# deryrahman/image-caption-emotion-indonesia

Measured on AMD Instinct MI355X. Metric: images/sec (train step) + NLL loss match, batch=64 ResNet152+FactoredLSTM-512, higher is better.
Workload: dtype f32 (trunk: operands as 2 f16 pieces each, 3 MFMA products per multiply, f32 accumulate; decoder: large products as 3 bf16 pieces per operand, 6 MFMA products per multiply, the rest f32 MFMA; the persistent LSTM kernel the trunk's split-f16 scheme)

## Files before the change

image-caption-emotion-indonesia_amd/_lib.py:

```python
import ctypes as C
import os

_HERE = os.path.dirname(os.path.abspath(__file__))
LIB_PATH = os.path.join(_HERE, "libcapnet_hip.so")

_f = C.POINTER(C.c_float)
_vp = C.c_void_p
_i = C.c_int
_l = C.c_long
_sz = C.c_size_t
_ip = C.POINTER(C.c_int)

SIGNATURES = {
    "capnet_last_error": (C.c_char_p, []),
    "capnet_abi_version": (_i, []),
    "capnet_sgemm": (_i, [_i, _i, _i, _i, _i, _vp, _l, _vp, _l, _vp, _l, _vp, _i, _i, _l, _l, _l,
                          _l, _i, _vp]),
    "capnet_sgemm_b3": (_i, [_i, _i, _i, _i, _i, _vp, _l, _vp, _l, _vp, _l, _vp, _i, _i, _l, _l, _l, _l, _vp, _sz, _vp]),
    "capnet_sgemm_b3_eligible": (_i, [_i, _i, _i, _i, _i, _vp, _l, _vp, _l, _vp, _l, _vp, _i, _l, _l, _l, _l]),
    "capnet_sgemm_splitk": (_i, [_i, _i, _i, _i, _i, _vp, _l, _vp, _l, _vp, _l, _vp, _i, _vp, _sz, _vp]),
    "capnet_sgemm_splitk_fused": (_i, [_i, _i, _i, _i, _i, _vp, _l, _vp, _l, _vp, _l, _vp, _i, _vp, _sz, _vp, _sz, _vp]),
    "capnet_colsum": (_i, [_vp, _l, _i, _i, _vp, _i, _vp]),
    "capnet_argmax_rows": (_i, [_vp, _i, _i, _i, _vp, _vp]),
    "capnet_resize_u8": (_i, [_vp, _i, _i, _vp, _vp, _i, _i, _vp, _vp, _i, _vp, _vp, _i, _vp]),
# ... 38 lines not shown
    "capnet_conv1x1_f16x3_weight_words": (_sz, [_i, _i]),
    "capnet_conv1x1_f16x3_bn": (_i, [_l, _i]),
    "capnet_conv1x1_f16x3_pack": (_i, [_vp, _vp, _i, _i, _i, _vp]),
    "capnet_conv1x1_fwd_f16x3": (_i, [_vp, _l, _l, _l, _vp, _i, _vp, _vp, _vp, _i, _vp, _vp, _i, _i, _i, _i, _i,
                                      _i, _vp, _vp, _vp, _i, _vp]),
    "capnet_conv3x3_fwd_patch": (_i, [_vp, _vp, _i, _vp, _vp, _vp, _i, _vp, _vp, _i, _i, _i, _i, _i, _i, _vp]),
    "capnet_conv1x1_fwd_tail": (_i, [_vp, _vp, _vp, _vp, _vp, _vp, _vp, _vp, _i, _vp, _vp, _vp, _l, _i, _i, _vp]),
    "capnet_conv2d_fwd_f16x3_scaled": (_i, [_vp, _l, _l, _l, _vp, _i, _vp, _vp, _vp, _i, _vp, _vp, _i, _i, _i, _i, _i,
                                            _i, _i, _i, _i, _vp]),
    "capnet_conv3x3_fwd_patch_scaled": (_i, [_vp, _vp, _i, _vp, _vp, _vp, _i, _vp, _vp, _i, _i, _i, _i, _i, _i, _i, _vp]),
    "capnet_conv1x1_fwd_tail_scaled": (_i, [_vp, _vp, _vp, _vp, _vp, _vp, _vp, _vp, _i, _vp, _vp, _vp, _l, _i, _i, _i, _vp]),
    "capnet_conv_stem_f16x3_weight_words": (_sz, []),
    "capnet_conv_stem_f16x3_part_rows": (_i, [_i, _i, _i]),
    "capnet_conv_stem_f16x3_pack": (_i, [_vp, _vp, _vp]),
    "capnet_conv_stem_fwd_f16x3": (_i, [_vp, _l, _l, _l, _vp, _vp, _vp, _vp, _i, _i, _i, _vp]),
    "capnet_conv_f16x3_weight_words": (_sz, [_i, _i, _i]),
    "capnet_conv_f16x3_pack": (_i, [_vp, _vp, _i, _i, _i, _i, _vp]),
    "capnet_conv2d_fwd_f16x3": (_i, [_vp, _l, _l, _l, _vp, _i, _vp, _vp, _vp, _i, _vp, _vp, _i, _i, _i, _i, _i,
                                     _i, _i, _i, _vp, _vp, _vp, _i, _vp]),
    "capnet_conv_kmajor_slab_floats": (_sz, [_i, _i, _i, _i]),
    "capnet_conv_kmajor_plan": (None, [_i, _i, _i, _i, _ip]),
    "capnet_conv_kmajor_tiles_m": (_i, [_i, _i, _i, _i]),
    "capnet_conv_tiles_m": (_i, [_i, _i, _i]),
    "capnet_bn_finalize": (_i, [_vp, _vp, _i, _i, _l, _vp, _vp, _vp, _vp, C.c_float, C.c_float,
                                _vp, _vp, _vp]),
    "capnet_bn_add_relu": (_i, [_vp, _vp, _vp, _vp, _vp, _vp, _vp, _l, _i, _vp]),
    "capnet_bn_relu_maxpool": (_i, [_vp, _vp, _vp, _vp, _i, _i, _i, _i, _vp]),
    "capnet_global_avgpool": (_i, [_vp, _vp, _i, _i, _i, _vp]),
    "capnet_bn1d_fwd": (_i, [_vp, _i, _i, _vp, _vp, _vp, _vp, _i, C.c_float, C.c_float, _vp, _vp,
                             _vp, _vp]),
# ... 210 lines not shown
```

image-caption-emotion-indonesia_amd/csrc/capi.cpp:

```cpp
#include "../../include/capnet.h"

#include "common.h"
#include "kernels.h"

using namespace capnet;

static inline hipStream_t S(capnet_stream_t s) { return reinterpret_cast<hipStream_t>(s); }

static SeqDims to_dims(const int* d) {
  SeqDims r;
  r.B = d[0]; r.T = d[1]; r.steps = d[2]; r.N = d[3]; r.E = d[4]; r.F = d[5]; r.H = d[6];
  r.V = d[7]; r.has_features = d[8]; r.cell = d[9];
  return r;
}

static bool weight_used(int cell, int i) { return cell == kCellFactored || i == 0 || i == 4 || i == 24 || i == 28; }
template <class Weights>
static void to_weights(const float* const* weights, Weights& w) {
  for (int g = 0; g < 4; ++g) {
    w.Vw[g] = weights[0 + g];  w.Vb[g] = weights[4 + g];
    w.Sw[g] = weights[8 + g];  w.Sb[g] = weights[12 + g];
    w.Uw[g] = weights[16 + g]; w.Ub[g] = weights[20 + g];
    w.Ww[g] = weights[24 + g]; w.Wb[g] = weights[28 + g];
  }
// ... 137 lines not shown
}
int capnet_conv1x1_fwd_tail_scaled(const float* y3, const float* s1, const float* t1, const float* res, const float* s2,
                                   const float* t2, float* tail_out, const unsigned* image, int bn, float* y,
                                   float* part_sum, float* part_sq, long M, int Cin, int Cout, int in_exp,
                                   capnet_stream_t stream) {
  return conv1x1_fwd_tail(y3, s1, t1, res, s2, t2, tail_out, image, bn, y, part_sum, part_sq, M, Cin, Cout, S(stream), in_exp);
}
size_t capnet_conv_stem_f16x3_weight_words(void) { return conv_stem_f16x3_weight_words(); }
int capnet_conv_stem_f16x3_part_rows(int B, int H, int W) { return conv_stem_f16x3_part_rows(B, H, W); }
int capnet_conv_stem_f16x3_pack(const float* w_oihw, unsigned* image, capnet_stream_t stream) {
  return conv_stem_f16x3_pack(w_oihw, image, S(stream));
}
int capnet_conv_stem_fwd_f16x3(const float* x, long sxb, long sxc, long sxh, const unsigned* image, float* y,
                               float* part_sum, float* part_sq, int B, int H, int W, capnet_stream_t stream) {
  return conv_stem_fwd_f16x3(x, sxb, sxc, sxh, image, y, part_sum, part_sq, B, H, W, S(stream));
}

int capnet_sgemm_splitk(int transA, int transB, int M, int N, int K, const float* A, long lda,
                        const float* B, long ldb, float* C, long ldc, const float* bias,
                        int accumulate, float* workspace, size_t workspace_floats,
                        capnet_stream_t stream) {
  CAPNET_REQUIRE(M >= 0 && N >= 0 && K >= 0, "sgemm_splitk: negative dimension");
  return sgemm_splitk(transA != 0, transB != 0, M, N, K, A, lda, B, ldb, C, ldc, bias, accumulate,
                      workspace, workspace_floats, S(stream));
}
int capnet_sgemm_splitk_fused(int transA, int transB, int M, int N, int K, const float* A, long lda,
                              const float* B, long ldb, float* C, long ldc, const float* bias,
                              int accumulate, float* workspace, size_t workspace_floats, int* counters,
                              size_t n_counters, capnet_stream_t stream) {
  CAPNET_REQUIRE(M >= 0 && N >= 0 && K >= 0, "sgemm_splitk_fused: negative dimension");
// ... 1083 lines not shown
```

image-caption-emotion-indonesia_amd/csrc/conv_stem.hip:

```cpp
#include <cstdlib>

#include "common.h"
#include "mfma_core.h"
#include "split_f16.h"
#include "kernels.h"

namespace capnet {
namespace {

constexpr int kRows = 22;
constexpr int kSteps = kRows / 2;
constexpr int kSeg = 128;
constexpr int kCols = 2 * kSeg + 8;
constexpr int kGroups = kCols / 4;
constexpr int kRowDw = 160;
constexpr int kPlane = kRows * kRowDw * 4;
constexpr int kImgBytes = 2 * kSteps * 2 * 64 * 16;
constexpr int kLoads = (21 * kGroups + 255) / 256;
constexpr int kWgs = 512;
static_assert(kRowDw * 2 >= kCols && kRowDw % 64 == 32, "staged row stride");

struct StemArgs {
  const float* x;
  const unsigned* wimg;
  float* y;
  float* part_sum;
  float* part_sq;
  int B, H, W, OH, OW, chunks, tiles, in_exp;
  int* err;
  int sxb, sxc, sxh;
  unsigned tile_mul, tile_sh;
  unsigned oh_mul, oh_sh;
};

__global__ __launch_bounds__(256, 2) void conv_stem_f16x3_kernel(const StemArgs g) {
  __shared__ __attribute__((aligned(16))) unsigned char lds[kImgBytes + 2 * kPlane];
  __shared__ float s_red[2][4][64];
  unsigned char* const wl = lds;
  unsigned char* const xl = lds + kImgBytes;
  const int tid = threadIdx.x, lane = tid & 63, wave = tid >> 6;
  const int li = lane & 31, lh = lane >> 5;
  const float oscale = f16x3_out_scale(g.wimg[0], g.in_exp);
  const float iscale = ldexpf(1.f, g.in_exp);

  {
    const u4* src = reinterpret_cast<const u4*>(g.wimg + kF16x3HdrWords);
    for (int i = tid; i < kImgBytes / 16; i += 256) *reinterpret_cast<u4*>(wl + i * 16) = src[i];
    for (int i = tid; i < kRowDw; i += 256) {
      *reinterpret_cast<unsigned*>(xl + (21 * kRowDw + i) * 4) = 0u;
      *reinterpret_cast<unsigned*>(xl + kPlane + (21 * kRowDw + i) * 4) = 0u;
    }
  }

  f32x4 pre[kLoads];
  auto fetch = [&](int tile) {
    const int boh = (int)fast_div((unsigned)tile, g.tile_mul, g.tile_sh), chunk = tile - boh * g.chunks;
    const int b = (int)fast_div((unsigned)boh, g.oh_mul, g.oh_sh), oh = boh - b * g.OH;
    const int iw0 = 2 * chunk * kSeg - 4;
#pragma unroll
    for (int u = 0; u < kLoads; ++u) {
      const int i = tid + 256 * u;
      const int r = i / kGroups, q = i - r * kGroups;
      const int c = r / 7, kh = r - 7 * c;
      const int ih = 2 * oh - 3 + kh, iw = iw0 + 4 * q;
      const bool ok = r < 21 && (unsigned)ih < (unsigned)g.H && iw >= 0 && iw < g.W;
      f32x4 v = {0.f, 0.f, 0.f, 0.f};
      if (ok) v = *reinterpret_cast<const f32x4*>(g.x + (long)b * g.sxb + (long)c * g.sxc + (long)ih * g.sxh + iw);
      pre[u] = v;
    }
  };
  auto stage = [&]() {
#pragma unroll
    for (int u = 0; u < kLoads; ++u) {
      const int i = tid + 256 * u;
      const int r = i / kGroups, q = i - r * kGroups;
      if (r < 21) {
        h4 h, l;
        split4(pre[u] * iscale, h, l);
        *reinterpret_cast<h4*>(xl + r * kRowDw * 4 + q * 8) = h;
        *reinterpret_cast<h4*>(xl + kPlane + r * kRowDw * 4 + q * 8) = l;
      }
    }
  };

  float csum[2] = {0.f, 0.f}, csq[2] = {0.f, 0.f};
  const int G = (int)gridDim.x;
  int tile = xcd_remap((int)blockIdx.x, G);
  if (tile < g.tiles) fetch(tile);
  __syncthreads();
  for (; tile < g.tiles; tile += G) {
    stage();
    __syncthreads();
    const int boh = (int)fast_div((unsigned)tile, g.tile_mul, g.tile_sh), chunk = tile - boh * g.chunks;
    if (tile + G < g.tiles) fetch(tile + G);
    f32x16 acc[2];
#pragma unroll
    for (int nb = 0; nb < 2; ++nb)
#pragma unroll
      for (int r = 0; r < 16; ++r) acc[nb][r] = 0.f;
    const unsigned char* arow = xl + (lh * kRowDw + 32 * wave + li) * 4;
    const unsigned char* brow = wl + (lh * 64 + li) * 16;
#pragma unroll
    for (int s = 0; s < kSteps; ++s) {
      h8 a[2], bf[2][2];
#pragma unroll
      for (int p = 0; p < 2; ++p) {
        const unsigned* ap = reinterpret_cast<const unsigned*>(arow + p * kPlane + s * 2 * kRowDw * 4);
        const u4 av = {ap[0], ap[1], ap[2], ap[3]};
        a[p] = __builtin_bit_cast(h8, av);
#pragma unroll
        for (int nb = 0; nb < 2; ++nb)
          bf[p][nb] = *reinterpret_cast<const h8*>(brow + ((p * kSteps + s) * 2 * 64 + nb * 32) * 16);
      }
#pragma unroll
      for (int nb = 0; nb < 2; ++nb) {
        acc[nb] = __builtin_amdgcn_mfma_f32_32x32x16_f16(a[1], bf[0][nb], acc[nb], 0, 0, 0);
        acc[nb] = __builtin_amdgcn_mfma_f32_32x32x16_f16(a[0], bf[1][nb], acc[nb], 0, 0, 0);
        acc[nb] = __builtin_amdgcn_mfma_f32_32x32x16_f16(a[0], bf[0][nb], acc[nb], 0, 0, 0);
      }
    }
    const int ow_base = chunk * kSeg + 32 * wave + 4 * lh;
    float* yrow = g.y + ((long)boh * g.OW) * 64;
#pragma unroll
    for (int nb = 0; nb < 2; ++nb) {
#pragma unroll
      for (int r = 0; r < 16; ++r) {
        const int ow = ow_base + (r & 3) + 8 * (r >> 2);
        const float v = acc[nb][r] * oscale;
        if (ow < g.OW) {
          yrow[(long)ow * 64 + nb * 32 + li] = v;
          csum[nb] += v;
          csq[nb] = fmaf(v, v, csq[nb]);
        }
      }
    }
    __syncthreads();
  }
  if (!g.part_sum && g.err) flag_nonfinite(csq[0] + csq[1], g.err);
  if (g.part_sum) {
#pragma unroll
    for (int nb = 0; nb < 2; ++nb) {
      csum[nb] += __shfl_xor(csum[nb], 32);
      csq[nb] += __shfl_xor(csq[nb], 32);
      if (lh == 0) {
        s_red[0][wave][nb * 32 + li] = csum[nb];
        s_red[1][wave][nb * 32 + li] = csq[nb];
      }
    }
    __syncthreads();
    if (tid < 64) {
      g.part_sum[(long)blockIdx.x * 64 + tid] = (s_red[0][0][tid] + s_red[0][1][tid]) + (s_red[0][2][tid] + s_red[0][3][tid]);
// ... 58 lines not shown
                        float* part_sq, int Bn, int H, int W, hipStream_t stream, int in_exp, int* err) {
  CAPNET_REQUIRE(x && wimg && y && aligned16(wimg) && in_exp > -64 && in_exp < 64, "conv_stem_fwd_f16x3: bad argument");
  CAPNET_REQUIRE(conv_stem_f16x3_eligible(x, sxb, sxc, sxh, 1, Bn, H, W, 3, 64, 7, 2, 3),
                 "conv_stem_fwd_f16x3: operands not eligible (B=%d %dx%d)", Bn, H, W);
  CAPNET_REQUIRE((part_sum == nullptr) == (part_sq == nullptr), "conv_stem_fwd_f16x3: stats pair");
  StemArgs a{};
  a.x = x; a.wimg = wimg; a.y = y; a.part_sum = part_sum; a.part_sq = part_sq;
  a.B = Bn; a.H = H; a.W = W; a.OH = (H - 1) / 2 + 1; a.OW = (W - 1) / 2 + 1;
  a.in_exp = in_exp; a.err = err;
  a.chunks = cdiv(a.OW, kSeg);
  a.tiles = Bn * a.OH * a.chunks;
  a.sxb = (int)sxb; a.sxc = (int)sxc; a.sxh = (int)sxh;
  magic_div((unsigned)a.chunks, &a.tile_mul, &a.tile_sh);
  magic_div((unsigned)a.OH, &a.oh_mul, &a.oh_sh);
  const int grid = a.tiles < kWgs ? a.tiles : kWgs;
  CAPNET_LAUNCH_TIMED(conv_stem_f16x3_kernel, dim3(grid), dim3(256), stream, a);
  CAPNET_LAUNCH_CHECK();
  return kOk;
}

}
```

image-caption-emotion-indonesia_amd/csrc/kernels.h:

```cpp
#pragma once
#include <hip/hip_runtime.h>

namespace capnet {

int sgemm(bool ta, bool tb, int M, int N, int K, const float* A, long lda, const float* B,
          long ldb, float* C, long ldc, const float* bias, int accumulate, int batch, long sA,
          long sB, long sC, long sBias, int force_tile, hipStream_t stream);

bool sgemm_b3_eligible(bool ta, bool tb, int M, int N, int K, const float* A, long lda, const float* B, long ldb,
                       const float* C, long ldc, const float* bias, int batch, long sA, long sB, long sC, long sBias);
int sgemm_b3(bool ta, bool tb, int M, int N, int K, const float* A, long lda, const float* B, long ldb, float* C, long ldc,
             const float* bias, int accumulate, int batch, long sA, long sB, long sC, long sBias, hipStream_t stream,
             float* ws = nullptr, size_t ws_floats = 0);

constexpr size_t kSplitKCounters = 1024;
int sgemm_splitk(bool ta, bool tb, int M, int N, int K, const float* A, long lda, const float* B,
                 long ldb, float* C, long ldc, const float* bias, int accumulate, float* ws,
                 size_t ws_floats, hipStream_t stream, int* counters = nullptr, size_t n_counters = 0);
int sgemm_splitk_slabs(bool tb, int M, int N, int K, const float* A, long lda, const float* B, long ldb,
                       float* ws, size_t ws_floats, int* n_slabs, hipStream_t stream);
int sgemm_rows16_slabs(bool tb, int M, int N, int K, const float* A, long lda, const float* B, long ldb, float* ws,
                       size_t ws_floats, int* n_slabs, hipStream_t stream);
int sgemm_splitk_batched(bool ta, bool tb, int M, int N, int K, const float* A, long lda,
                         const float* B, long ldb, float* C, long ldc, const float* bias,
// ... 37 lines not shown
size_t conv_f16x3_weight_words(int Cin, int Cout, int k);
int f16x3_pack_header(const float* w, unsigned* img, long n, hipStream_t stream);
int conv_f16x3_pack(const float* w_oihw, unsigned* img, int Cout, int Cin, int k, int bn, hipStream_t stream);
int conv_fwd_f16x3(const float* x, long sxb, long sxh, long sxw, const unsigned* wimg, int bn, float* y,
                   const float* in_scale, const float* in_shift, int relu_in, float* part_sum, float* part_sq, int Bn,
                   int H, int W, int Cin, int Cout, int k, int stride, int pad, hipStream_t stream,
                   const float* out_scale = nullptr, const float* out_shift = nullptr, const float* res = nullptr,
                   int relu_out = 0, int in_exp = 0, int* err = nullptr);
bool conv_stem_f16x3_eligible(const float* x, long sxb, long sxc, long sxh, long sxw, int Bn, int H, int W, int Cin,
                              int Cout, int k, int stride, int pad);
size_t conv_stem_f16x3_weight_words();
int conv_stem_f16x3_part_rows(int Bn, int H, int W);
int conv_stem_f16x3_pack(const float* w_oihw, unsigned* img, hipStream_t stream);
int conv_stem_fwd_f16x3(const float* x, long sxb, long sxc, long sxh, const unsigned* wimg, float* y, float* part_sum,
                        float* part_sq, int Bn, int H, int W, hipStream_t stream, int in_exp = 0, int* err = nullptr);
bool conv3x3_patch_eligible(const float* x, long sxb, long sxh, long sxw, long sxc, int Bn, int H, int W, int Cin,
                            int Cout, int k, int stride, int pad, const float* in_scale, const float* in_shift);
int conv3x3_fwd_patch(const float* x, const unsigned* wimg, int bn, float* y, const float* in_scale, const float* in_shift,
                      int relu_in, float* part_sum, float* part_sq, int Bn, int H, int W, int Cin, int Cout,
                      hipStream_t stream, bool shared_chip = false, int in_exp = 0, int* err = nullptr);
bool conv1x1_areg_eligible(const float* x, long M, int Cin, int Cout, int bn, const float* in_scale, const float* in_shift);
int conv1x1_fwd_areg(const float* x, const unsigned* wimg, int bn, float* y, const float* in_scale, const float* in_shift,
                     int relu_in, float* part_sum, float* part_sq, long M, int Cin, int Cout, int in_exp, hipStream_t stream,
                     int* err = nullptr);
bool conv1x1_tail_eligible(const float* y3, const float* res, long M, int Cin, int Cout);
int conv1x1_fwd_tail(const float* y3, const float* s1, const float* t1, const float* res, const float* s2, const float* t2,
                     float* tail_out, const unsigned* wimg, int bn, float* y, float* part_sum, float* part_sq, long M,
                     int Cin, int Cout, hipStream_t stream, int in_exp = 0, int* err = nullptr);
size_t conv1x1_f16x3_weight_words(int Cin, int Cout);
int conv1x1_f16x3_pack(const float* w, unsigned* img, int Cout, int Cin, int bn, hipStream_t stream);
// ... 382 lines not shown
```

image-caption-emotion-indonesia_amd/csrc/trunk.cpp:

```cpp
#include <algorithm>
#include <cstdint>
#include <cstdlib>
#include <cstring>
#include <cstdio>
#include <utility>
#include <vector>

#include "common.h"
#include "kernels.h"

namespace capnet {

struct TrunkConv {
  int Cin, Cout, k, stride, pad;
  int H, W;
  int OH, OW;
  int Kw;
  bool kmajor;
  bool h3;
  int tile_n;
  bool stem_h3 = false;
  bool fused3 = false, fused1 = false;
};

// ... 1 lines not shown
  int stage, index;
  int i1, i2, i3, id;
};

struct Trunk {
  int B, H, W;
  std::vector<TrunkConv> convs;
  std::vector<TrunkBlock> blocks;
  size_t off_x[2], off_y1, off_y2, off_y3, off_d, off_part, off_slab, off_gram, off_ss, total_floats;
  std::vector<size_t> ss_off;
  std::vector<size_t> bs_off;
  int final_side;
  bool tail_balance = true;
  bool use_patch = true, fuse_tails = true, use_areg = false;
  int fused_stages = 0;
  bool timing = false;
  int timing_every = 1;
  long pass_no = 0;
  bool timing_now = false;
  bool timing_once = false;
  std::vector<hipEvent_t> ev_pool;
  size_t ev_next = 0;
  std::vector<hipEvent_t> ev;
  double timed_flops = 0;
};

static int round_up(int v, int m) { return (v + m - 1) / m * m; }
static const float* const kAlignedDummy = reinterpret_cast<const float*>(uintptr_t(256));

int trunk_create(int B, int H, int W, Trunk** out) {
// ... 68 lines not shown
      max_y1 = std::max(max_y1, (size_t)c1.OH * c1.OW * c1.Cout);
      max_y2 = std::max(max_y2, (size_t)c2.OH * c2.OW * c2.Cout);
      max_y3 = std::max(max_y3, (size_t)c3.OH * c3.OW * c3.Cout);
      t->blocks.push_back(TrunkBlock{L, b, i1, i1 + 1, i1 + 2, b == 0 ? i1 + 3 : -1});
      if (b == 0) {
        TrunkConv d = add(inplanes, p * 4, 1, stride, 0, h, w, true);
        max_d = std::max(max_d, (size_t)d.OH * d.OW * d.Cout);
      }
      h = c2.OH; w = c2.OW;
      inplanes = p * 4;
      max_x = std::max(max_x, (size_t)h * w * inplanes);
    }
  }
  t->final_side = h;
  CAPNET_REQUIRE(h == w, "trunk_create: only square feature maps are supported");
  max_y3 = std::max(max_y3, (size_t)stem.OH * stem.OW * 64);
  size_t off = 0;
  auto take = [&](size_t n) { size_t o = off; off += (n + 63) / 64 * 64; return o; };
  t->off_x[0] = take(max_x * B);
  t->off_x[1] = take(max_x * B);
  t->off_y1 = take(max_y1 * B);
  t->off_y2 = take(max_y2 * B);
  t->off_y3 = take(max_y3 * B);
  t->off_d = take(max_d * B);
  size_t max_part = 0;
  for (auto& c : t->convs) {
    const long M = (long)B * c.OH * c.OW;
    const int tile = c.kmajor ? conv_v2_auto_tile((int)M, c.Cout, c.Kw) : conv_auto_tile((int)M, c.Cout);
    max_part = std::max(max_part, (size_t)conv_tiles_m((int)M, tile) * c.Cout);
    if (c.h3) max_part = std::max(max_part, (size_t)conv1x1_tiles_m(M) * c.Cout);
    if (c.stem_h3) max_part = std::max(max_part, (size_t)conv_stem_f16x3_part_rows(B, c.H, c.W) * c.Cout);
  }
  max_part = std::max(max_part, max_fpart);
  t->off_part = take(2 * max_part);
  size_t max_slab = 0;
  for (auto& c : t->convs)
    if (c.kmajor) max_slab = std::max(max_slab, conv_v2_slab_floats(B * c.OH * c.OW, c.Cout, c.Kw, 0));
  t->off_slab = take(max_slab + 64);
  t->off_gram = take(max_gram + 64);
  t->off_ss = off;
  for (auto& c : t->convs) t->ss_off.push_back(take(2 * (size_t)c.Cout));
  for (auto& c : t->convs) t->bs_off.push_back(take(2 * (size_t)c.Cout));
  t->total_floats = off;
  *out = t;
  return kOk;
}
// ... 187 lines not shown
int conv_bn(const Ctx& c, int i, const float* x, long sxb, long sxh, long sxw, long sxc,
            const float* in_scale, const float* in_shift, int relu_in, float* y, const BlockTail* tail = nullptr) {
  const TrunkConv& d = c.t->convs[i];
  const long M = (long)c.t->B * d.OH * d.OW;
  CAPNET_REQUIRE(d.tile_n != 256 || d.k == 3 || (tail && (c.train || c.eval_ready)), "trunk: conv %d was planned for the wide tail kernel", i);
  const bool fuse_tail = tail && (c.train || c.eval_ready) && c.t->fuse_tails && d.h3 && d.k == 1 && d.stride == 1 && !in_scale &&
                         x == tail->out && tail->C == d.Cin && tail->rows == M && sxc == 1 && sxw == d.Cin &&
                         sxh == (long)d.W * d.Cin && sxb == (long)d.H * d.W * d.Cin &&
                         conv1x1_tail_eligible(tail->y3, tail->res, M, d.Cin, d.Cout);
  if (tail && !fuse_tail) {
    const int rt = run_tail(c, *tail);
    if (rt) return rt;
  }
  int tile = d.kmajor ? conv_v2_auto_tile((int)M, d.Cout, d.Kw) : conv_auto_tile((int)M, d.Cout);
  if (d.kmajor && !c.t->tail_balance && M >= 5000) tile = 12864;
  const int prows = d.stem_h3 ? conv_stem_f16x3_part_rows(c.t->B, d.H, d.W) : d.h3 ? conv1x1_tiles_m(M) : conv_tiles_m((int)M, tile);
  float* psum = c.ws + c.t->off_part;
  float* psq = psum + (size_t)prows * d.Cout;
  const bool attach = fuse_tail || d.stem_h3 || d.h3;
  const int rc = timed_launch(c.t, attach, c.s, trunk_conv_flops(c.t, i), [&]() -> int {
    const unsigned* wimg = reinterpret_cast<const unsigned*>(c.w[i]);
    float* ps = c.train ? psum : nullptr;
    float* pq = c.train ? psq : nullptr;
    if (fuse_tail)
      return conv1x1_fwd_tail(tail->y3, tail->s1, tail->t1, tail->res, tail->s2, tail->t2, tail->out, wimg, d.tile_n, y, ps, pq, M,
                              d.Cin, d.Cout, c.s, c.in_exp(i), c.err);
    if (d.stem_h3) {
      CAPNET_REQUIRE(!in_scale && conv_stem_f16x3_eligible(x, sxb, sxc, sxh, sxw, c.t->B, d.H, d.W, d.Cin, d.Cout, d.k, d.stride, d.pad),
                     "trunk: the stem is planned for the split-f16 kernel but its operands are not eligible");
      return conv_stem_fwd_f16x3(x, sxb, sxc, sxh, wimg, y, ps, pq, c.t->B, d.H, d.W, c.s, c.in_exp(i), c.err);
    }
    if (d.h3 && d.k == 3 && c.t->use_patch &&
        conv3x3_patch_eligible(x, sxb, sxh, sxw, sxc, c.t->B, d.H, d.W, d.Cin, d.Cout, d.k, d.stride, d.pad, in_scale, in_shift))
      return conv3x3_fwd_patch(x, wimg, d.tile_n, y, in_scale, in_shift, relu_in, ps, pq, c.t->B, d.H, d.W, d.Cin, d.Cout, c.s,
                               !c.t->tail_balance, c.in_exp(i), c.err);
    if (d.h3 && d.k == 1 && d.stride == 1 && c.t->use_areg && sxc == 1 && sxw == d.Cin && sxh == (long)d.W * d.Cin &&
        sxb == (long)d.H * d.W * d.Cin && conv1x1_areg_eligible(x, M, d.Cin, d.Cout, d.tile_n, in_scale, in_shift))
      return conv1x1_fwd_areg(x, wimg, d.tile_n, y, in_scale, in_shift, relu_in, ps, pq, M, d.Cin, d.Cout, c.in_exp(i), c.s, c.err);
    if (d.h3) {
      CAPNET_REQUIRE(conv_f16x3_eligible(x, sxb, sxh, sxw, sxc, c.t->B, d.H, d.W, d.Cin, d.Cout, d.k, d.stride, d.pad, in_scale, in_shift),
                     "trunk: conv %d planned for the split-f16 kernel but its operands are not eligible", i);
      return conv_fwd_f16x3(x, sxb, sxh, sxw, wimg, d.tile_n, y, in_scale, in_shift, relu_in, ps, pq, c.t->B, d.H, d.W, d.Cin, d.Cout,
                            d.k, d.stride, d.pad, c.s, nullptr, nullptr, nullptr, 0, c.in_exp(i), c.err);
    }
// ... 153 lines not shown
  float* Y1 = workspace + t->off_y1;
  float* Y2 = workspace + t->off_y2;
  float* Y3 = workspace + t->off_y3;
  float* D = workspace + t->off_d;
  int rc;
  if (!train) {
    const char* fe = getenv("CAPNET_EVAL_FOLDED");
    if (fe && fe[0] == '1') return trunk_forward_eval(c, images_nchw, out_pooled, out_map);
    rc = eval_scale_shift_all(c);
    if (rc) return rc;
    c.eval_ready = true;
  }
  {
    const TrunkConv& d = t->convs[0];
    rc = conv_bn(c, 0, images_nchw, (long)3 * d.H * d.W, d.W, 1, (long)d.H * d.W, nullptr,
                 nullptr, 0, Y3);
    if (rc) return rc;
    rc = bn_relu_maxpool(Y3, c.scale(0), c.shift(0), X[0], B, d.OH, d.OW, 64, stream);
    if (rc) return rc;
  }
  int cur = 0;
  BlockTail tail{};
  FusedTail ftail{};
  bool have_tail = false, have_ftail = false;
  for (const TrunkBlock& blk : t->blocks) {
    const int i1 = blk.i1, i2 = blk.i2, i3 = blk.i3, id = blk.id;
    const TrunkConv& c1 = t->convs[i1];
    const TrunkConv& c2 = t->convs[i2];
    const TrunkConv& c3 = t->convs[i3];
    const float* x = X[cur];
    float* out = X[cur ^ 1];
    auto nhwc = [](const TrunkConv& d, long* sb, long* sh, long* sw) {
      *sw = d.Cin; *sh = (long)d.W * d.Cin; *sb = (long)d.H * d.W * d.Cin;
    };
    long sb, sh, sw;
    nhwc(c1, &sb, &sh, &sw);
    if (have_ftail) {
      CAPNET_REQUIRE(c1.fused1 && (c.train || c.eval_ready), "trunk: conv %d is not the fused boundary the plan made", i1);
      rc = fused_conv1_bn(c, i1, ftail, Y1);
      have_ftail = false;
    } else {
      CAPNET_REQUIRE(!c1.fused1, "trunk: conv %d was planned for fused_block.hip", i1);
      rc = conv_bn(c, i1, x, sb, sh, sw, 1, nullptr, nullptr, 0, Y1, have_tail ? &tail : nullptr);
    }
    have_tail = false;
    if (rc) return rc;
    nhwc(c2, &sb, &sh, &sw);
    rc = conv_bn(c, i2, Y1, sb, sh, sw, 1, c.scale(i1), c.shift(i1), 1, Y2);
    if (rc) return rc;
    const long rows = (long)B * c3.OH * c3.OW;
    if (c3.fused3 && (c.train || c.eval_ready)) {
      rc = fused_stats_bn(c, i3, Y2, c.scale(i2), c.shift(i2));
      if (rc) return rc;
      if (id >= 0) {
        const TrunkConv& cd = t->convs[id];
        nhwc(cd, &sb, &sh, &sw);
        rc = conv_bn(c, id, x, sb, sh, sw, 1, nullptr, nullptr, 0, D);
        if (rc) return rc;
        ftail = FusedTail{i3, Y2, c.scale(i2), c.shift(i2), D, c.scale(id), c.shift(id), out};
      } else {
        ftail = FusedTail{i3, Y2, c.scale(i2), c.shift(i2), x, nullptr, nullptr, out};
      }
      have_ftail = true;
      cur ^= 1;
      continue;
    }
    CAPNET_REQUIRE(!c3.fused3, "trunk: conv %d was planned for fused_block.hip (the folded inference trunk must be chosen before the plan is made)", i3);
    nhwc(c3, &sb, &sh, &sw);
    rc = conv_bn(c, i3, Y2, sb, sh, sw, 1, c.scale(i2), c.shift(i2), 1, Y3);
    if (rc) return rc;
    if (id >= 0) {
      const TrunkConv& cd = t->convs[id];
      nhwc(cd, &sb, &sh, &sw);
      rc = conv_bn(c, id, x, sb, sh, sw, 1, nullptr, nullptr, 0, D);
      if (rc) return rc;
      tail = BlockTail{Y3, c.scale(i3), c.shift(i3), D, c.scale(id), c.shift(id), out, rows, c3.Cout};
    } else {
      tail = BlockTail{Y3, c.scale(i3), c.shift(i3), x, nullptr, nullptr, out, rows, c3.Cout};
    }
    have_tail = true;
    cur ^= 1;
  }
  if (have_tail) {
    rc = run_tail(c, tail);
    if (rc) return rc;
  }
  const int side = t->final_side;
  if (out_pooled) {
    rc = global_avgpool(X[cur], out_pooled, B, side * side, 2048, stream, c.err);
// ... 11 lines not shown
```

include/capnet.h:

```cpp
#ifndef CAPNET_H_
#define CAPNET_H_

#include <stddef.h>

#ifdef __cplusplus
extern "C" {
#endif

typedef void* capnet_stream_t;
typedef struct capnet_trunk capnet_trunk_t;

#define CAPNET_OK 0
#define CAPNET_ERR_INVALID_ARG (-1)
#define CAPNET_ERR_HIP (-2)

const char* capnet_last_error(void);
int capnet_abi_version(void);

int capnet_sgemm(int transA, int transB, int M, int N, int K, const float* A, long lda,
                 const float* B, long ldb, float* C, long ldc, const float* bias, int accumulate,
                 int batch, long strideA, long strideB, long strideC, long strideBias,
                 int force_tile, capnet_stream_t stream);
int capnet_sgemm_b3(int transA, int transB, int M, int N, int K, const float* A, long lda, const float* B, long ldb,
                    float* C, long ldc, const float* bias, int accumulate, int batch, long strideA, long strideB,
// ... 118 lines not shown
                                   float* part_sq, int B, int H, int W, int Cin, int Cout, int k, int stride, int pad,
                                   int in_exp, capnet_stream_t stream);
int capnet_conv3x3_fwd_patch_scaled(const float* x, const unsigned* image, int bn, float* y, const float* in_scale,
                                    const float* in_shift, int relu_in, float* part_sum, float* part_sq, int B, int H,
                                    int W, int Cin, int Cout, int shared_chip, int in_exp, capnet_stream_t stream);
int capnet_conv1x1_fwd_tail_scaled(const float* y3, const float* s1, const float* t1, const float* res, const float* s2,
                                   const float* t2, float* tail_out, const unsigned* image, int bn, float* y,
                                   float* part_sum, float* part_sq, long M, int Cin, int Cout, int in_exp,
                                   capnet_stream_t stream);

size_t capnet_conv_stem_f16x3_weight_words(void);
int capnet_conv_stem_f16x3_part_rows(int B, int H, int W);
int capnet_conv_stem_f16x3_pack(const float* w_oihw, unsigned* image, capnet_stream_t stream);
int capnet_conv_stem_fwd_f16x3(const float* x, long sxb, long sxc, long sxh, const unsigned* image, float* y,
                               float* part_sum, float* part_sq, int B, int H, int W, capnet_stream_t stream);

int capnet_conv2d_fwd_kmajor(const float* x, long sxb, long sxh, long sxw, const float* w_kmajor,
                             int k_rows, float* y, const float* in_scale, const float* in_shift,
                             int relu_in, float* part_sum, float* part_sq, int B, int H, int W,
                             int Cin, int Cout, int KH, int KW, int stride, int pad, int tile,
                             float* slabs, capnet_stream_t stream);
size_t capnet_conv_kmajor_slab_floats(int M, int Cout, int k_rows, int tile);
void capnet_conv_kmajor_plan(int M, int Cout, int k_rows, int tile, int* out5);
int capnet_conv_kmajor_tiles_m(int M, int Cout, int k_rows, int tile);
int capnet_conv_tiles_m(int M, int Cout, int tile);
int capnet_bn_finalize(const float* part_sum, const float* part_sq, int tiles, int C, long count,
                       const float* gamma, const float* beta, float* running_mean,
                       float* running_var, float momentum, float eps, float* scale, float* shift,
                       capnet_stream_t stream);
int capnet_bn_add_relu(const float* y, const float* s1, const float* t1, const float* res,
// ... 349 lines not shown
```

Measured before the change: 9208.

## Fuse stem conv with max-pool and defer BN-ReLU into first block convs

Adds a pooled variant of the split-f16 stem kernel that max-pools each output row pair in registers (sign-flipped by gamma so max commutes with the BN affine) and writes only the pooled map, while still gathering BN statistics. The separate BN+ReLU+maxpool pass and the full-resolution stem output round trip are dropped; the BN scale/shift and ReLU are instead applied on input by the first bottleneck's 1x1 and downsample convs. Work units are runs of pooled rows per image, which changes the stem's parallel decomposition and adds overlap rows and an extra LDS sync per row. It is on by default when eligible and can be disabled by env var. Forward trunk only.

```diff
diff --git a/image-caption-emotion-indonesia_amd/_lib.py b/image-caption-emotion-indonesia_amd/_lib.py
--- a/image-caption-emotion-indonesia_amd/_lib.py
+++ b/image-caption-emotion-indonesia_amd/_lib.py
@@ -76,6 +76,9 @@
     "capnet_conv_stem_f16x3_part_rows": (_i, [_i, _i, _i]),
     "capnet_conv_stem_f16x3_pack": (_i, [_vp, _vp, _vp]),
     "capnet_conv_stem_fwd_f16x3": (_i, [_vp, _l, _l, _l, _vp, _vp, _vp, _vp, _i, _i, _i, _vp]),
+    "capnet_conv_stem_pool_f16x3_eligible": (_i, [_vp, _l, _l, _l, _i, _i, _i]),
+    "capnet_conv_stem_pool_f16x3_part_rows": (_i, [_i, _i, _i]),
+    "capnet_conv_stem_pool_fwd_f16x3": (_i, [_vp, _l, _l, _l, _vp, _vp, _vp, _vp, _vp, _i, _i, _i, _i, _vp]),
     "capnet_conv_f16x3_weight_words": (_sz, [_i, _i, _i]),
     "capnet_conv_f16x3_pack": (_i, [_vp, _vp, _i, _i, _i, _i, _vp]),
     "capnet_conv2d_fwd_f16x3": (_i, [_vp, _l, _l, _l, _vp, _i, _vp, _vp, _vp, _i, _vp, _vp, _i, _i, _i, _i, _i,
diff --git a/image-caption-emotion-indonesia_amd/csrc/capi.cpp b/image-caption-emotion-indonesia_amd/csrc/capi.cpp
--- a/image-caption-emotion-indonesia_amd/csrc/capi.cpp
+++ b/image-caption-emotion-indonesia_amd/csrc/capi.cpp
@@ -175,6 +175,15 @@
 int capnet_conv_stem_fwd_f16x3(const float* x, long sxb, long sxc, long sxh, const unsigned* image, float* y,
                                float* part_sum, float* part_sq, int B, int H, int W, capnet_stream_t stream) {
   return conv_stem_fwd_f16x3(x, sxb, sxc, sxh, image, y, part_sum, part_sq, B, H, W, S(stream));
+}
+int capnet_conv_stem_pool_f16x3_eligible(const float* x, long sxb, long sxc, long sxh, int B, int H, int W) {
+  return conv_stem_pool_f16x3_eligible(x, sxb, sxc, sxh, 1, B, H, W, 3, 64, 7, 2, 3) ? 1 : 0;
+}
+int capnet_conv_stem_pool_f16x3_part_rows(int B, int H, int W) { return conv_stem_pool_f16x3_part_rows(B, H, W); }
+int capnet_conv_stem_pool_fwd_f16x3(const float* x, long sxb, long sxc, long sxh, const unsigned* image, const float* gamma,
+                                    float* pooled, float* part_sum, float* part_sq, int B, int H, int W, int in_exp,
+                                    capnet_stream_t stream) {
+  return conv_stem_pool_fwd_f16x3(x, sxb, sxc, sxh, image, gamma, pooled, part_sum, part_sq, B, H, W, S(stream), in_exp);
 }
 
 int capnet_sgemm_splitk(int transA, int transB, int M, int N, int K, const float* A, long lda,
diff --git a/image-caption-emotion-indonesia_amd/csrc/conv_stem.hip b/image-caption-emotion-indonesia_amd/csrc/conv_stem.hip
--- a/image-caption-emotion-indonesia_amd/csrc/conv_stem.hip
+++ b/image-caption-emotion-indonesia_amd/csrc/conv_stem.hip
@@ -18,6 +18,7 @@
 constexpr int kImgBytes = 2 * kSteps * 2 * 64 * 16;
 constexpr int kLoads = (21 * kGroups + 255) / 256;
 constexpr int kWgs = 512;
+constexpr int kPoolRun = 7;
 static_assert(kRowDw * 2 >= kCols && kRowDw % 64 == 32, "staged row stride");
 
 struct StemArgs {
@@ -31,11 +32,16 @@
   int sxb, sxc, sxh;
   unsigned tile_mul, tile_sh;
   unsigned oh_mul, oh_sh;
+  const float* gamma;
+  int PH, PW, run, upi;
+  unsigned upi_mul, upi_sh;
 };
 
+template <bool POOL>
 __global__ __launch_bounds__(256, 2) void conv_stem_f16x3_kernel(const StemArgs g) {
   __shared__ __attribute__((aligned(16))) unsigned char lds[kImgBytes + 2 * kPlane];
   __shared__ float s_red[2][4][64];
+  __shared__ float s_edge[POOL ? 4 : 1][64];
   unsigned char* const wl = lds;
   unsigned char* const xl = lds + kImgBytes;
   const int tid = threadIdx.x, lane = tid & 63, wave = tid >> 6;
@@ -53,9 +59,7 @@
   }
 
   f32x4 pre[kLoads];
-  auto fetch = [&](int tile) {
-    const int boh = (int)fast_div((unsigned)tile, g.tile_mul, g.tile_sh), chunk = tile - boh * g.chunks;
-    const int b = (int)fast_div((unsigned)boh, g.oh_mul, g.oh_sh), oh = boh - b * g.OH;
+  auto fetch_row = [&](int b, int oh, int chunk) {
     const int iw0 = 2 * chunk * kSeg - 4;
 #pragma unroll
     for (int u = 0; u < kLoads; ++u) {
@@ -69,6 +73,11 @@
       pre[u] = v;
     }
   };
+  auto fetch = [&](int tile) {
+    const int boh = (int)fast_div((unsigned)tile, g.tile_mul, g.tile_sh), chunk = tile - boh * g.chunks;
+    const int b = (int)fast_div((unsigned)boh, g.oh_mul, g.oh_sh), oh = boh - b * g.OH;
+    fetch_row(b, oh, chunk);
+  };
   auto stage = [&]() {
 #pragma unroll
     for (int u = 0; u < kLoads; ++u) {
@@ -83,17 +92,7 @@
     }
   };
 
-  float csum[2] = {0.f, 0.f}, csq[2] = {0.f, 0.f};
-  const int G = (int)gridDim.x;
-  int tile = xcd_remap((int)blockIdx.x, G);
-  if (tile < g.tiles) fetch(tile);
-  __syncthreads();
-  for (; tile < g.tiles; tile += G) {
-    stage();
-    __syncthreads();
-    const int boh = (int)fast_div((unsigned)tile, g.tile_mul, g.tile_sh), chunk = tile - boh * g.chunks;
-    if (tile + G < g.tiles) fetch(tile + G);
-    f32x16 acc[2];
+  auto product = [&](f32x16 (&acc)[2]) {
 #pragma unroll
     for (int nb = 0; nb < 2; ++nb)
 #pragma unroll
@@ -119,22 +118,159 @@
         acc[nb] = __builtin_amdgcn_mfma_f32_32x32x16_f16(a[0], bf[0][nb], acc[nb], 0, 0, 0);
       }
     }
-    const int ow_base = chunk * kSeg + 32 * wave + 4 * lh;
-    float* yrow = g.y + ((long)boh * g.OW) * 64;
-#pragma unroll
-    for (int nb = 0; nb < 2; ++nb) {
-#pragma unroll
-      for (int r = 0; r < 16; ++r) {
-        const int ow = ow_base + (r & 3) + 8 * (r >> 2);
-        const float v = acc[nb][r] * oscale;
-        if (ow < g.OW) {
-          yrow[(long)ow * 64 + nb * 32 + li] = v;
-          csum[nb] += v;
-          csq[nb] = fmaf(v, v, csq[nb]);
+  };
+
+  float csum[2] = {0.f, 0.f}, csq[2] = {0.f, 0.f};
+  const int G = (int)gridDim.x;
+  int tile = xcd_remap((int)blockIdx.x, G);
+  if constexpr (!POOL) {
+    if (tile < g.tiles) fetch(tile);
+    __syncthreads();
+    for (; tile < g.tiles; tile += G) {
+      stage();
+      __syncthreads();
+      const int boh = (int)fast_div((unsigned)tile, g.tile_mul, g.tile_sh), chunk = tile - boh * g.chunks;
+      if (tile + G < g.tiles) fetch(tile + G);
+      f32x16 acc[2];
+      product(acc);
+      const int ow_base = chunk * kSeg + 32 * wave + 4 * lh;
+      float* yrow = g.y + ((long)boh * g.OW) * 64;
+#pragma unroll
+      for (int nb = 0; nb < 2; ++nb) {
+#pragma unroll
+        for (int r = 0; r < 16; ++r) {
+          const int ow = ow_base + (r & 3) + 8 * (r >> 2);
+          const float v = acc[nb][r] * oscale;
+          if (ow < g.OW) {
+            yrow[(long)ow * 64 + nb * 32 + li] = v;
+            csum[nb] += v;
+            csq[nb] = fmaf(v, v, csq[nb]);
+          }
         }
       }
+      __syncthreads();
+    }
+  } else {
+    auto open_unit = [&](int unit, int& b, int& oh, int& end) {
+      b = (int)fast_div((unsigned)unit, g.upi_mul, g.upi_sh);
+      const int ph0 = (unit - b * g.upi) * g.run;
+      oh = ph0 > 0 ? 2 * ph0 - 1 : 0;
+      end = min(2 * (ph0 + g.run), g.OH);
+    };
+    const float kNone = -__builtin_inff();
+    float sgn[2];
+#pragma unroll
+    for (int nb = 0; nb < 2; ++nb) sgn[nb] = (g.gamma && g.gamma[nb * 32 + li] < 0.f) ? -1.f : 1.f;
+    const float osgn[2] = {oscale * sgn[0], oscale * sgn[1]};
+    float vm[2][8];
+    int b = 0, oh = 0, end = 0;
+    bool fresh = true;
+    if (tile < g.tiles) {
+      open_unit(tile, b, oh, end);
+      fetch_row(b, oh, 0);
     }
     __syncthreads();
+    while (tile < g.tiles) {
+      stage();
+      __syncthreads();
+      int ntile = tile, nb_ = b, noh = oh + 1, nend = end;
+      if (noh == end) {
+        ntile = tile + G;
+        if (ntile < g.tiles) open_unit(ntile, nb_, noh, nend);
+      }
+      if (ntile < g.tiles) fetch_row(nb_, noh, 0);
+      f32x16 acc[2];
+      product(acc);
+      const bool owned = !(fresh && (oh & 1));
+      const int lim = g.OW - (32 * wave + 4 * lh);
+#pragma unroll
+      for (int nb = 0; nb < 2; ++nb)
+#pragma unroll
+        for (int r = 0; r < 16; ++r) acc[nb][r] *= osgn[nb];
+      if (owned) {
+#pragma unroll
+        for (int k = 0; k < 4; ++k) {
+          if (8 * k + 3 < lim) {
+#pragma unroll
+            for (int nb = 0; nb < 2; ++nb)
+#pragma unroll
+              for (int j = 0; j < 4; ++j) {
+                csum[nb] += acc[nb][4 * k + j];
+                csq[nb] = fmaf(acc[nb][4 * k + j], acc[nb][4 * k + j], csq[nb]);
+              }
+          } else if (8 * k < lim) {
+#pragma unroll
+            for (int nb = 0; nb < 2; ++nb)
+#pragma unroll
+              for (int j = 0; j < 3; ++j)
+                if (8 * k + j < lim) {
+                  csum[nb] += acc[nb][4 * k + j];
+                  csq[nb] = fmaf(acc[nb][4 * k + j], acc[nb][4 * k + j], csq[nb]);
+                }
+          }
+        }
+      }
+      if (g.OW & 1) {
+#pragma unroll
+        for (int nb = 0; nb < 2; ++nb)
+#pragma unroll
+          for (int k = 0; k < 4; ++k) {
+            if (8 * k + 1 == lim) acc[nb][4 * k + 1] = kNone;
+            if (8 * k + 3 == lim) acc[nb][4 * k + 3] = kNone;
+          }
+      }
+#pragma unroll
+      for (int nb = 0; nb < 2; ++nb)
+        if (lh) s_edge[wave][nb * 32 + li] = acc[nb][15];
+      __syncthreads();
+      float hm[2][8];
+#pragma unroll
+      for (int nb = 0; nb < 2; ++nb) {
+        float t[4];
+#pragma unroll
+        for (int k = 0; k < 4; ++k) t[k] = __shfl_xor(acc[nb][4 * k + 3], 32);
+        const float e = wave > 0 ? s_edge[wave - 1][nb * 32 + li] : kNone;
+#pragma unroll
+        for (int k = 0; k < 4; ++k) {
+          const float left = lh ? t[k] : (k ? t[k > 0 ? k - 1 : 0] : e);
+          hm[nb][2 * k] = fmaxf(fmaxf(left, acc[nb][4 * k]), acc[nb][4 * k + 1]);
+          hm[nb][2 * k + 1] = fmaxf(fmaxf(acc[nb][4 * k + 1], acc[nb][4 * k + 2]), acc[nb][4 * k + 3]);
+        }
+      }
+      auto store_row = [&](const float (&v)[2][8]) {
+        float* prow = g.y + (((long)b * g.PH + (oh >> 1)) * g.PW) * 64;
+#pragma unroll
+        for (int nb = 0; nb < 2; ++nb)
+#pragma unroll
+          for (int j = 0; j < 8; ++j) {
+            const int pw = 16 * wave + 4 * (j >> 1) + 2 * lh + (j & 1);
+            if (pw < g.PW) prow[(long)pw * 64 + nb * 32 + li] = v[nb][j] * sgn[nb];
+          }
+      };
+      if (oh & 1) {
+        if (owned) {
+#pragma unroll
+          for (int nb = 0; nb < 2; ++nb)
+#pragma unroll
+            for (int j = 0; j < 8; ++j) vm[nb][j] = fmaxf(vm[nb][j], hm[nb][j]);
+          store_row(vm);
+        }
+#pragma unroll
+        for (int nb = 0; nb < 2; ++nb)
+#pragma unroll
+          for (int j = 0; j < 8; ++j) vm[nb][j] = hm[nb][j];
+      } else {
+#pragma unroll
+        for (int nb = 0; nb < 2; ++nb)
+#pragma unroll
+          for (int j = 0; j < 8; ++j) vm[nb][j] = fresh ? hm[nb][j] : fmaxf(vm[nb][j], hm[nb][j]);
+        if (oh == g.OH - 1) store_row(vm);
+      }
+      fresh = ntile != tile;
+      tile = ntile; b = nb_; oh = noh; end = nend;
+    }
+    csum[0] *= sgn[0];
+    csum[1] *= sgn[1];
   }
   if (!g.part_sum && g.err) flag_nonfinite(csq[0] + csq[1], g.err);
   if (g.part_sum) {
@@ -223,9 +359,50 @@
   magic_div((unsigned)a.chunks, &a.tile_mul, &a.tile_sh);
   magic_div((unsigned)a.OH, &a.oh_mul, &a.oh_sh);
   const int grid = a.tiles < kWgs ? a.tiles : kWgs;
-  CAPNET_LAUNCH_TIMED(conv_stem_f16x3_kernel, dim3(grid), dim3(256), stream, a);
+  CAPNET_LAUNCH_TIMED(conv_stem_f16x3_kernel<false>, dim3(grid), dim3(256), stream, a);
   CAPNET_LAUNCH_CHECK();
   return kOk;
 }
 
-}
+namespace {
+long stem_pool_units(int Bn, int H) {
+  const long PH = ((H - 1) / 2 + 1 - 1) / 2 + 1;
+  return (long)Bn * cdiv(PH, PH < kPoolRun ? PH : (long)kPoolRun);
+}
+}
+bool conv_stem_pool_f16x3_eligible(const float* x, long sxb, long sxc, long sxh, long sxw, int Bn, int H, int W, int Cin,
+                                   int Cout, int k, int stride, int pad) {
+  return conv_stem_f16x3_eligible(x, sxb, sxc, sxh, sxw, Bn, H, W, Cin, Cout, k, stride, pad) && (W - 1) / 2 + 1 <= kSeg &&
+         stem_pool_units(Bn, H) < (1l << 24);
+}
+int conv_stem_pool_f16x3_part_rows(int Bn, int H, int W) {
+  (void)W;
+  const long units = stem_pool_units(Bn, H);
+  return (int)(units < kWgs ? units : kWgs);
+}
+
+int conv_stem_pool_fwd_f16x3(const float* x, long sxb, long sxc, long sxh, const unsigned* wimg, const float* gamma,
+                             float* pooled, float* part_sum, float* part_sq, int Bn, int H, int W, hipStream_t stream,
+                             int in_exp, int* err) {
+  CAPNET_REQUIRE(x && wimg && pooled && aligned16(wimg) && in_exp > -64 && in_exp < 64, "conv_stem_pool_fwd_f16x3: bad argument");
+  CAPNET_REQUIRE(conv_stem_pool_f16x3_eligible(x, sxb, sxc, sxh, 1, Bn, H, W, 3, 64, 7, 2, 3),
+                 "conv_stem_pool_fwd_f16x3: operands not eligible (B=%d %dx%d)", Bn, H, W);
+  CAPNET_REQUIRE((part_sum == nullptr) == (part_sq == nullptr), "conv_stem_pool_fwd_f16x3: stats pair");
+  StemArgs a{};
+  a.x = x; a.wimg = wimg; a.y = pooled; a.part_sum = part_sum; a.part_sq = part_sq; a.gamma = gamma;
+  a.B = Bn; a.H = H; a.W = W; a.OH = (H - 1) / 2 + 1; a.OW = (W - 1) / 2 + 1;
+  a.PH = (a.OH - 1) / 2 + 1; a.PW = (a.OW - 1) / 2 + 1;
+  a.in_exp = in_exp; a.err = err;
+  a.chunks = 1;
+  a.run = a.PH < kPoolRun ? a.PH : kPoolRun;
+  a.upi = cdiv(a.PH, a.run);
+  a.tiles = Bn * a.upi;
+  a.sxb = (int)sxb; a.sxc = (int)sxc; a.sxh = (int)sxh;
+  magic_div((unsigned)a.upi, &a.upi_mul, &a.upi_sh);
+  const int grid = a.tiles < kWgs ? a.tiles : kWgs;
+  CAPNET_LAUNCH_TIMED(conv_stem_f16x3_kernel<true>, dim3(grid), dim3(256), stream, a);
+  CAPNET_LAUNCH_CHECK();
+  return kOk;
+}
+
+}
diff --git a/image-caption-emotion-indonesia_amd/csrc/kernels.h b/image-caption-emotion-indonesia_amd/csrc/kernels.h
--- a/image-caption-emotion-indonesia_amd/csrc/kernels.h
+++ b/image-caption-emotion-indonesia_amd/csrc/kernels.h
@@ -75,6 +75,12 @@
 int conv_stem_f16x3_pack(const float* w_oihw, unsigned* img, hipStream_t stream);
 int conv_stem_fwd_f16x3(const float* x, long sxb, long sxc, long sxh, const unsigned* wimg, float* y, float* part_sum,
                         float* part_sq, int Bn, int H, int W, hipStream_t stream, int in_exp = 0, int* err = nullptr);
+bool conv_stem_pool_f16x3_eligible(const float* x, long sxb, long sxc, long sxh, long sxw, int Bn, int H, int W, int Cin,
+                                   int Cout, int k, int stride, int pad);
+int conv_stem_pool_f16x3_part_rows(int Bn, int H, int W);
+int conv_stem_pool_fwd_f16x3(const float* x, long sxb, long sxc, long sxh, const unsigned* wimg, const float* gamma,
+                             float* pooled, float* part_sum, float* part_sq, int Bn, int H, int W, hipStream_t stream,
+                             int in_exp = 0, int* err = nullptr);
 bool conv3x3_patch_eligible(const float* x, long sxb, long sxh, long sxw, long sxc, int Bn, int H, int W, int Cin,
                             int Cout, int k, int stride, int pad, const float* in_scale, const float* in_shift);
 int conv3x3_fwd_patch(const float* x, const unsigned* wimg, int bn, float* y, const float* in_scale, const float* in_shift,
diff --git a/image-caption-emotion-indonesia_amd/csrc/trunk.cpp b/image-caption-emotion-indonesia_amd/csrc/trunk.cpp
--- a/image-caption-emotion-indonesia_amd/csrc/trunk.cpp
+++ b/image-caption-emotion-indonesia_amd/csrc/trunk.cpp
@@ -39,6 +39,7 @@
   bool tail_balance = true;
   bool use_patch = true, fuse_tails = true, use_areg = false;
   int fused_stages = 0;
+  bool stem_pool = false;
   bool timing = false;
   int timing_every = 1;
   long pass_no = 0;
@@ -137,6 +138,12 @@
   }
   t->final_side = h;
   CAPNET_REQUIRE(h == w, "trunk_create: only square feature maps are supported");
+  {
+    const TrunkBlock& b0 = t->blocks.front();
+    t->stem_pool = t->convs[0].stem_h3 && !env_on("CAPNET_NO_STEM_POOL") && b0.id >= 0 && t->convs[b0.i1].h3 &&
+                   t->convs[b0.id].h3 && !t->convs[b0.i1].fused1 &&
+                   conv_stem_pool_f16x3_eligible(kAlignedDummy, (long)3 * H * W, (long)H * W, W, 1, B, H, W, 3, 64, 7, 2, 3);
+  }
   max_y3 = std::max(max_y3, (size_t)stem.OH * stem.OW * 64);
   size_t off = 0;
   auto take = [&](size_t n) { size_t o = off; off += (n + 63) / 64 * 64; return o; };
@@ -153,6 +160,7 @@
     max_part = std::max(max_part, (size_t)conv_tiles_m((int)M, tile) * c.Cout);
     if (c.h3) max_part = std::max(max_part, (size_t)conv1x1_tiles_m(M) * c.Cout);
     if (c.stem_h3) max_part = std::max(max_part, (size_t)conv_stem_f16x3_part_rows(B, c.H, c.W) * c.Cout);
+    if (c.stem_h3 && t->stem_pool) max_part = std::max(max_part, (size_t)conv_stem_pool_f16x3_part_rows(B, c.H, c.W) * c.Cout);
   }
   max_part = std::max(max_part, max_fpart);
   t->off_part = take(2 * max_part);
@@ -370,7 +378,8 @@
   }
   int tile = d.kmajor ? conv_v2_auto_tile((int)M, d.Cout, d.Kw) : conv_auto_tile((int)M, d.Cout);
   if (d.kmajor && !c.t->tail_balance && M >= 5000) tile = 12864;
-  const int prows = d.stem_h3 ? conv_stem_f16x3_part_rows(c.t->B, d.H, d.W) : d.h3 ? conv1x1_tiles_m(M) : conv_tiles_m((int)M, tile);
+  const bool pool = d.stem_h3 && c.t->stem_pool;
+  const int prows = pool ? conv_stem_pool_f16x3_part_rows(c.t->B, d.H, d.W) : d.stem_h3 ? conv_stem_f16x3_part_rows(c.t->B, d.H, d.W) : d.h3 ? conv1x1_tiles_m(M) : conv_tiles_m((int)M, tile);
   float* psum = c.ws + c.t->off_part;
   float* psq = psum + (size_t)prows * d.Cout;
   const bool attach = fuse_tail || d.stem_h3 || d.h3;
@@ -384,6 +393,11 @@
     if (d.stem_h3) {
       CAPNET_REQUIRE(!in_scale && conv_stem_f16x3_eligible(x, sxb, sxc, sxh, sxw, c.t->B, d.H, d.W, d.Cin, d.Cout, d.k, d.stride, d.pad),
                      "trunk: the stem is planned for the split-f16 kernel but its operands are not eligible");
+      if (pool) {
+        CAPNET_REQUIRE(conv_stem_pool_f16x3_eligible(x, sxb, sxc, sxh, sxw, c.t->B, d.H, d.W, d.Cin, d.Cout, d.k, d.stride, d.pad),
+                       "trunk: the stem is planned for the pooled kernel but its operands are not eligible");
+        return conv_stem_pool_fwd_f16x3(x, sxb, sxc, sxh, wimg, c.gamma[i], y, ps, pq, c.t->B, d.H, d.W, c.s, c.in_exp(i), c.err);
+      }
       return conv_stem_fwd_f16x3(x, sxb, sxc, sxh, wimg, y, ps, pq, c.t->B, d.H, d.W, c.s, c.in_exp(i), c.err);
     }
     if (d.h3 && d.k == 3 && c.t->use_patch &&
@@ -567,11 +581,15 @@
   {
     const TrunkConv& d = t->convs[0];
     rc = conv_bn(c, 0, images_nchw, (long)3 * d.H * d.W, d.W, 1, (long)d.H * d.W, nullptr,
-                 nullptr, 0, Y3);
-    if (rc) return rc;
-    rc = bn_relu_maxpool(Y3, c.scale(0), c.shift(0), X[0], B, d.OH, d.OW, 64, stream);
-    if (rc) return rc;
-  }
+                 nullptr, 0, t->stem_pool ? X[0] : Y3);
+    if (rc) return rc;
+    if (!t->stem_pool) {
+      rc = bn_relu_maxpool(Y3, c.scale(0), c.shift(0), X[0], B, d.OH, d.OW, 64, stream);
+      if (rc) return rc;
+    }
+  }
+  const float* s0 = t->stem_pool ? c.scale(0) : nullptr;
+  const float* t0 = t->stem_pool ? c.shift(0) : nullptr;
   int cur = 0;
   BlockTail tail{};
   FusedTail ftail{};
@@ -583,6 +601,10 @@
     const TrunkConv& c3 = t->convs[i3];
     const float* x = X[cur];
     float* out = X[cur ^ 1];
+    const bool first = &blk == &t->blocks.front();
+    const float* xs = first ? s0 : nullptr;
+    const float* xt = first ? t0 : nullptr;
+    const int xrelu = xs ? 1 : 0;
     auto nhwc = [](const TrunkConv& d, long* sb, long* sh, long* sw) {
       *sw = d.Cin; *sh = (long)d.W * d.Cin; *sb = (long)d.H * d.W * d.Cin;
     };
@@ -594,7 +616,7 @@
       have_ftail = false;
     } else {
       CAPNET_REQUIRE(!c1.fused1, "trunk: conv %d was planned for fused_block.hip", i1);
-      rc = conv_bn(c, i1, x, sb, sh, sw, 1, nullptr, nullptr, 0, Y1, have_tail ? &tail : nullptr);
+      rc = conv_bn(c, i1, x, sb, sh, sw, 1, xs, xt, xrelu, Y1, have_tail ? &tail : nullptr);
     }
     have_tail = false;
     if (rc) return rc;
@@ -608,7 +630,7 @@
       if (id >= 0) {
         const TrunkConv& cd = t->convs[id];
         nhwc(cd, &sb, &sh, &sw);
-        rc = conv_bn(c, id, x, sb, sh, sw, 1, nullptr, nullptr, 0, D);
+        rc = conv_bn(c, id, x, sb, sh, sw, 1, xs, xt, xrelu, D);
         if (rc) return rc;
         ftail = FusedTail{i3, Y2, c.scale(i2), c.shift(i2), D, c.scale(id), c.shift(id), out};
       } else {
@@ -625,7 +647,7 @@
     if (id >= 0) {
       const TrunkConv& cd = t->convs[id];
       nhwc(cd, &sb, &sh, &sw);
-      rc = conv_bn(c, id, x, sb, sh, sw, 1, nullptr, nullptr, 0, D);
+      rc = conv_bn(c, id, x, sb, sh, sw, 1, xs, xt, xrelu, D);
       if (rc) return rc;
       tail = BlockTail{Y3, c.scale(i3), c.shift(i3), D, c.scale(id), c.shift(id), out, rows, c3.Cout};
     } else {
diff --git a/include/capnet.h b/include/capnet.h
--- a/include/capnet.h
+++ b/include/capnet.h
@@ -156,6 +156,11 @@
 int capnet_conv_stem_f16x3_pack(const float* w_oihw, unsigned* image, capnet_stream_t stream);
 int capnet_conv_stem_fwd_f16x3(const float* x, long sxb, long sxc, long sxh, const unsigned* image, float* y,
                                float* part_sum, float* part_sq, int B, int H, int W, capnet_stream_t stream);
+int capnet_conv_stem_pool_f16x3_eligible(const float* x, long sxb, long sxc, long sxh, int B, int H, int W);
+int capnet_conv_stem_pool_f16x3_part_rows(int B, int H, int W);
+int capnet_conv_stem_pool_fwd_f16x3(const float* x, long sxb, long sxc, long sxh, const unsigned* image, const float* gamma,
+                                    float* pooled, float* part_sum, float* part_sq, int B, int H, int W, int in_exp,
+                                    capnet_stream_t stream);
 
 int capnet_conv2d_fwd_kmajor(const float* x, long sxb, long sxh, long sxw, const float* w_kmajor,
                              int k_rows, float* y, const float* in_scale, const float* in_shift,
```

After: 9299, median of 6. About the same (+1.0%).
